# bentherien/point-cloud-reid

Measured on NVIDIA B200. Metric: pair scores/sec (PT-256 encode + all-pairs xcorr_eff match), higher is better.
Workload: dtype f16

## Files before the change

include/pcreid.h:

```cpp
#ifndef PCREID_H_
#define PCREID_H_

#ifdef __cplusplus
extern "C" {
#endif

#define PCREID_OK 0
#define PCREID_ERR_ARG 1
#define PCREID_ERR_LAUNCH 2
#define PCREID_ERR_UNSUPPORTED 3

int pcreid_abi_version(void);


int pcreid_fps(int b, int n, int m, const float* xyz, float* temp, int* idx, void* stream);
int pcreid_fps_with_dist(int b, int n, int m, const float* dist, float* temp, int* idx, void* stream);
int pcreid_fps_block_size(int n);
int pcreid_fps_torch(int b, int n, int m, const float* xyz, const int* start, int* idx, void* stream);
int pcreid_pairwise_sqdist(int b, int n, int m, int c, const float* a, const float* bm, float* out, int norm, void* stream);

int pcreid_knn(int b, int n, int m, int nsample, const float* xyz, const float* new_xyz, int* idx, float* dist2, void* stream);
int pcreid_knn_t(int b, int n, int m, int nsample, const float* xyz, const float* new_xyz, int* idx, float* dist2, void* stream);

int pcreid_ball_query(int b, int n, int m, float min_radius, float max_radius, int nsample,
// ... 70 lines not shown
                   int rows2, const float* X2, long long x2_bs, int ldx2,
                   int mode, float* out, long long ob, long long oc, void* stream);
int pcreid_cn_chanmax(int B, int C, int rows, const float* X, long long x_bs, int ldx, float* out, long long ob, long long on, void* stream);

int pcreid_sa_edge_mlp(int B, int C, int N, int S, int k, const float* P1, const float* Cc, const int* idx,
                       const float* W2, const float* b2, const float* W3, const float* b3, float* out, void* stream);

int pcreid_edge_build(int B, int C, int N, int S, int k, const float* P1, const float* Cc, const int* idx, float* out, void* stream);
int pcreid_seg_max(long long rows, int k, const float* x, float* out, void* stream);
int pcreid_seg_mean(long long rows, int k, const float* x, float* out, void* stream);

int pcreid_edge_gather_max(int B, int C, int N, int k, const float* P, const float* Q, const int* idx, int act,
                           float* out, long long o_bs, int ldo, void* stream);

int pcreid_pair_concat_head_tc(int T, int D, int E, int G, const float* A, const float* Bv, const float* Et, const float* Ed,
                               const void* W2img, const float* g1, const float* be1, const float* g2, const float* be2,
                               const float* w, float b0, const unsigned char* mask, float* out, int n_ctas, void* stream);
int pcreid_pair_concat_head(int T, int D, int E, int G, const float* A, const float* Bv, const float* Et, const float* Ed,
                            const float* W2, const float* g1, const float* be1, const float* g2, const float* be2,
                            const float* w, float b0, const unsigned char* mask, float* out, void* stream);

#define PCREID_FMT_BF16 0
#define PCREID_FMT_F16 1
int pcreid_pack_image(int B, int C, int N, const float* src, long long s_bs, int lds, int act, int fmt, void* dst, void* stream);
int pcreid_pack_image_bias(int B, int C, int N, const float* src, long long s_bs, int lds, const float* bias, int fmt, void* dst,
                           void* stream);
int pcreid_pack_b7(int B, const float* M, const float* ksum, int fmt, void* dst, void* stream);
int pcreid_pool_finish2(int P, int npts, const float* part, const float* bias , float* out, void* stream);
int pcreid_pair_p1a2(int n_units, int npts, int role, int fmt, float att_eps, const int* u_search, const int* u_templ,
                     const int* u_slot, const void* QF1, const void* H, const void* MK1, const void* W, void* A_out,
                     int n_ctas, void* stream);
int pcreid_pair_p1b_n(int n_units, int npts, int role, int fmt, float kv_scale, const int* u_search, const int* u_templ,
                      const int* u_slot, const void* PV, const void* W, void* A_out, void* B7_out, int n_ctas, void* stream);
int pcreid_pair_p2y(int n_units, int npts, int role, int fmt, float att_eps, const int* u_slot, const void* A_in, const void* B7_in,
                    const void* W, float* pool_part, int n_ctas, void* stream);

int pcreid_sa_edge_mlp_tc(int B, int C, int N, int S, int k, const float* P1, const float* Cc, const int* idx,
                          const float* W2img, const float* b2, const float* W3img, const float* b3, float* out,
                          int n_ctas, void* stream);

int pcreid_sa_edge_mlp_tc2(int B, int C, int N, int S, int k, const float* P1, const float* Cc, const int* idx,
                           const float* W2img, const float* b2, const float* W3img, const float* b3, float* out,
                           int out_pm, int n_sms, void* stream);

int pcreid_attn_front_blob_bytes(int C2, int DP, int NFP, int NF);
int pcreid_attn_front(int B, int S, int C2, int DP, int NFP, int NF, const float* xyz, const float* feat, long long f_bs, int ldf,
                      const float* wp0, const float* bp0, const float* bp2, const void* blob, float* out, long long o_bs, int ldo,
                      void* stream);
int pcreid_linattn_kv_img(int B, int S, int d, int H, const float* K, long long k_bs, int ldk, const float* V, long long v_bs, int ldv,
                          float* kvimg, float* ksum, void* stream);
int pcreid_attn_back_objects_per_tile(int rows, int D);
int pcreid_attn_back_blob_bytes(int D, int C1P, int CO, int qpre);
int pcreid_attn_back(int B, int rows, int D, int H, int C1, int CO, int res, int f1_pm, const float* feat1, long long f1_bs,
                     int ldf1, const float* q, long long q_bs, int ldq, const float* ksum, const float* kvimg, const float* g1,
                     const float* b1, const float* g2, const float* b2, const void* blob, float* out, long long o_bs, int ldo,
                     void* stream);

#ifdef __cplusplus
}
#endif
#endif
```

point-cloud-reid_b200/_lib.py:

```python
import ctypes
import os

_HERE = os.path.dirname(os.path.abspath(__file__))
LIB_PATH = os.path.join(_HERE, "libpcreid_sm100.so")
_lib = None

c_int, c_ll, c_float, c_vp = ctypes.c_int, ctypes.c_longlong, ctypes.c_float, ctypes.c_void_p


class LinearArgs(ctypes.Structure):
    _fields_ = [
        ("B", c_int), ("rows", c_int), ("CO", c_int), ("K1", c_int), ("K2", c_int),
        ("X1", c_vp), ("x1_bs", c_ll), ("ldx1", c_int), ("x1_pm", c_int), ("x1_map", c_vp),
        ("X2", c_vp), ("x2_bs", c_ll), ("ldx2", c_int), ("x2_pm", c_int), ("x2_map", c_vp),
        ("W1", c_vp), ("w1_bs", c_ll), ("w1_map", c_vp),
        ("W2", c_vp), ("w2_bs", c_ll),
        ("bias", c_vp),
        ("R", c_vp), ("r_bs", c_ll), ("ldr", c_int), ("r_map", c_vp), ("res_after_act", c_int),
        ("act", c_int),
        ("Y", c_vp), ("y_bs", c_ll), ("ldy", c_int), ("y_pm", c_int),
    ]


class NormArgs(ctypes.Structure):
# ... 29 lines not shown
    "pcreid_crop_gather": [c_int, c_int, c_int, c_vp, c_int, c_vp, c_vp, c_vp, c_vp, c_vp, c_vp],
    "pcreid_three_nn": [c_int, c_int, c_int, c_vp, c_vp, c_vp, c_vp, c_vp],
    "pcreid_three_interpolate": [c_int, c_int, c_int, c_int, c_vp, c_vp, c_vp, c_vp, c_vp],
    "pcreid_cn_linear": [ctypes.POINTER(LinearArgs), c_vp],
    "pcreid_cn_linear_tc": [ctypes.POINTER(LinearArgs), c_vp],
    "pcreid_cn_linear_tc2": [ctypes.POINTER(LinearArgs), c_vp, c_vp, c_int, c_vp],
    "pcreid_cn_linear_tma": [ctypes.POINTER(LinearArgs), c_ll, c_ll, c_ll, c_int, c_int, c_vp],
    "pcreid_cn_linear_tma_x3": [ctypes.POINTER(LinearArgs), c_vp, c_vp, c_ll, c_ll, c_ll, c_int, c_vp],
    "pcreid_cn_groupnorm": [ctypes.POINTER(NormArgs), c_vp],
    "pcreid_gn_res_relu_dot": [c_int, c_int, c_int, c_vp, c_int, c_vp, c_vp, c_vp, c_int, c_vp, c_float, c_vp, c_vp],
    "pcreid_attn_front_blob_bytes": [c_int, c_int, c_int, c_int],
    "pcreid_attn_front": [c_int, c_int, c_int, c_int, c_int, c_int, c_vp, c_vp, c_ll, c_int, c_vp, c_vp, c_vp, c_vp, c_vp, c_ll, c_int,
                          c_vp],
    "pcreid_linattn_kv_img": [c_int, c_int, c_int, c_int, c_vp, c_ll, c_int, c_vp, c_ll, c_int, c_vp, c_vp, c_vp],
    "pcreid_attn_back_objects_per_tile": [c_int, c_int],
    "pcreid_attn_back_blob_bytes": [c_int, c_int, c_int, c_int],
    "pcreid_attn_back": [c_int] * 8 + [c_vp, c_ll, c_int, c_vp, c_ll, c_int] + [c_vp] * 7 + [c_vp, c_ll, c_int, c_vp],
    "pcreid_linattn_kv": [c_int, c_int, c_int, c_int, c_vp, c_ll, c_int, c_vp, c_ll, c_int, c_vp, c_vp, c_vp],
    "pcreid_linattn_scale": [c_int, c_int, c_int, c_int, c_int, c_vp, c_ll, c_int, c_vp, c_vp, c_vp, c_vp, c_ll, c_int, c_vp],
    "pcreid_local_linattn": [c_int, c_int, c_int, c_int, c_int, c_vp, c_vp, c_vp, c_vp],
    "pcreid_cn_pool": [c_int, c_int, c_int, c_vp, c_ll, c_int, c_int, c_vp, c_ll, c_int, c_int, c_vp, c_ll, c_ll, c_vp],
    "pcreid_cn_chanmax": [c_int, c_int, c_int, c_vp, c_ll, c_int, c_vp, c_ll, c_ll, c_vp],
    "pcreid_sa_edge_mlp": [c_int, c_int, c_int, c_int, c_int, c_vp, c_vp, c_vp, c_vp, c_vp, c_vp, c_vp, c_vp, c_vp],
    "pcreid_edge_build": [c_int, c_int, c_int, c_int, c_int, c_vp, c_vp, c_vp, c_vp, c_vp],
    "pcreid_seg_max": [c_ll, c_int, c_vp, c_vp, c_vp],
    "pcreid_seg_mean": [c_ll, c_int, c_vp, c_vp, c_vp],
    "pcreid_edge_gather_max": [c_int, c_int, c_int, c_int, c_vp, c_vp, c_vp, c_int, c_vp, c_ll, c_int, c_vp],
    "pcreid_pack_image": [c_int, c_int, c_int, c_vp, c_ll, c_int, c_int, c_int, c_vp, c_vp],
    "pcreid_pack_image_bias": [c_int, c_int, c_int, c_vp, c_ll, c_int, c_vp, c_int, c_vp, c_vp],
    "pcreid_pack_b7": [c_int, c_vp, c_vp, c_int, c_vp, c_vp],
    "pcreid_pool_finish2": [c_int, c_int, c_vp, c_vp, c_vp, c_vp],
    "pcreid_pair_p1a2": [c_int, c_int, c_int, c_int, c_float] + [c_vp] * 8 + [c_int, c_vp],
    "pcreid_pair_p1b_n": [c_int, c_int, c_int, c_int, c_float] + [c_vp] * 7 + [c_int, c_vp],
    "pcreid_pair_p2y": [c_int, c_int, c_int, c_int, c_float] + [c_vp] * 5 + [c_int, c_vp],
    "pcreid_sa_edge_mlp_tc": [c_int, c_int, c_int, c_int, c_int] + [c_vp] * 8 + [c_int, c_vp],
    "pcreid_sa_edge_mlp_tc2": [c_int, c_int, c_int, c_int, c_int] + [c_vp] * 8 + [c_int, c_int, c_vp],
    "pcreid_pair_concat_head_tc": [c_int, c_int, c_int, c_int] + [c_vp] * 10 + [c_float, c_vp, c_vp, c_int, c_vp],
    "pcreid_pair_concat_head": [c_int, c_int, c_int, c_int] + [c_vp] * 10 + [c_float, c_vp, c_vp, c_vp],
}

ERRORS = {1: "PCREID_ERR_ARG (bad pointer/size)", 2: "PCREID_ERR_LAUNCH (CUDA launch failed)",
          3: "PCREID_ERR_UNSUPPORTED (shape outside the built kernels)"}


def exported_symbols():
    return sorted(_SIGS.keys())


def lib():
    global _lib
    if _lib is not None:
        return _lib
    if not os.path.exists(LIB_PATH):
        from . import build as _build
        _build.build_library()
    if not os.path.exists(LIB_PATH):
        raise RuntimeError(f"{LIB_PATH} is missing and could not be built: the CUDA extension is required "
                           "(no CPU fallback exists)")
    L = ctypes.CDLL(LIB_PATH)
    for name, argt in _SIGS.items():
        fn = getattr(L, name)
        fn.argtypes = argt
        fn.restype = c_int
    _lib = L
    return L

# ... 10 lines not shown
```

point-cloud-reid_b200/csrc/pair_common.cuh:

```cuda
#pragma once
#include "../../include/pcreid.h"
#include "common.cuh"
#include "tc_common.cuh"

namespace {


constexpr int IMG = 16384;
constexpr int NB7H = 80;
constexpr int B7_HEAD = (NB7H / 8) * 32 * 16;
constexpr int B7_BYTES = 2 * B7_HEAD;
constexpr int ONES_BYTES = 2 * 2048;
constexpr float LN_EPS = 1e-5f;

struct P1Args {
  int n_units, NT, role;
  int npts;
  float att_eps;
  float kv_scale;
  const int *u_search, *u_templ, *u_slot;
  const uint8_t *QF1, *H, *PV;
  const uint8_t* MK1;
  const uint8_t* W;
  uint8_t* A_out;
  uint8_t* B7_out;
};
struct P2Args {
  int n_units, NT, role;
  int npts;
  float att_eps;
  const int* u_slot;
  const uint8_t* A_in;
  const uint8_t* B7_in;
  const uint8_t* W;
  float* pool_part;
};

__device__ __forceinline__ float elu1(float x) { return x > 0.f ? x + 1.f : __expf(x); }

__device__ __forceinline__ uint4 ldg_early(const void* p) {
  uint4 v;
  asm volatile("ld.global.nc.L1::no_allocate.v4.u32 {%0,%1,%2,%3}, [%4];" : "=r"(v.x), "=r"(v.y), "=r"(v.z), "=r"(v.w) : "l"(p));
  return v;
}

__device__ __forceinline__ void prefetch_l2_16k(const uint8_t* img, int t) {
  asm volatile("prefetch.global.L2 [%0];" ::"l"(img + (size_t)t * 128));
}

__device__ __forceinline__ void copy_to_smem(uint8_t* dst, const uint8_t* __restrict__ src, int bytes, int t, int nthr) {
  for (int i = t * 16; i < bytes; i += nthr * 16) cp_async16(dst + i, src + i);
}

struct Opnd {
  uint64_t desc;
  uint32_t kstep;
};
__device__ __forceinline__ Opnd opnd(uint32_t addr, uint32_t lbo, uint32_t sbo, uint32_t kstep_bytes) {
// ... 42 lines not shown
  uint32_t tmem, tlane;
  uint64_t* bar;
  uint32_t par;
  __device__ __forceinline__ void sync() { tc::bar_sync(1 + gid, GX); }
  __device__ __forceinline__ void publish() { tc::fence_async_smem(); tc::tc_fence_before(); sync(); tc::tc_fence_after(); }
  __device__ __forceinline__ void wait() { tc::mbar_wait(bar, par); par ^= 1u; tc::tc_fence_after(); }
};

__device__ __forceinline__ void ld32_stats(uint32_t taddr, float (&o)[32], float& s, float& ss) {
#pragma unroll
  for (int half = 0; half < 2; ++half) {
    uint32_t r[16];
    tc::tmem_ld16(taddr + 16 * half, r);
    tc::tmem_ld_wait();
#pragma unroll
    for (int j = 0; j < 16; ++j) {
      const float v = __uint_as_float(r[j]);
      o[16 * half + j] = v;
      s += v;
      ss = fmaf(v, v, ss);
    }
  }
}

template <class F>
__device__ __forceinline__ void write_b7_row(const float (&M)[64], float ksum, int d, uint8_t* dst) {
  float lo[32], hi[32];
#pragma unroll
  for (int j = 0; j < 32; ++j) { lo[j] = M[j]; hi[j] = M[32 + j]; }
  write_b7_part<F>(lo, 0, ksum, true, d, dst);
  write_b7_part<F>(hi, 4, ksum, false, d, dst);
}

__device__ __forceinline__ void groupx_setup(GroupX& g, uint64_t* bars, uint32_t tmem_base) {
  const int warp_u = (int)tc::uniform(threadIdx.x >> 5);
  g.gid = warp_u / 4;
  g.t = threadIdx.x % GX;
  g.issuer = (warp_u % 4) == 0;
  g.tmem = tc::uniform(tmem_base) + g.gid * 160;
  g.tlane = g.tmem + ((uint32_t)((warp_u % 4) * 32) << 16);
  g.bar = bars + g.gid;
  g.par = 0;
}

}
```

point-cloud-reid_b200/csrc/pair_tc.cu:

```cuda
#include "pair_common.cuh"
#include <stdlib.h>

namespace {

constexpr int P1B_WKV = 0, P1B_WM = 16384, P1B_WBYTES = 24576;
constexpr int P1B_AIMG = 0, P1B_KFV = IMG, P1B_GBYTES = IMG + 2 * IMG + ONES_BYTES;

template <class F, int CS>
__global__ void __launch_bounds__(NGX * GX * CS, 1) pair_p1b_kernel(const P1Args a) {
  constexpr int GT = GX * CS, NTHR = NGX * GT;
  constexpr int QB = 4 / CS, CB = 8 / CS;
  extern __shared__ __align__(1024) uint8_t smem[];
  __shared__ uint64_t bars[2 * NGX];
  __shared__ uint32_t tmem_base_s;
  uint8_t* Wsm = smem;
  if (threadIdx.x == 0) {
    for (int i = 0; i < 2 * NGX; ++i) tc::mbar_init(&bars[i], 1);
    tc::fence_mbar_init();
  }
  if (threadIdx.x < 32) { tc::tmem_alloc(&tmem_base_s, 512); tc::tmem_relinquish(); }
  copy_to_smem(Wsm, a.W, P1B_WBYTES, threadIdx.x, NTHR);
  cp_async_commit();
  cp_async_wait<0>();
  tc::fence_async_smem();
  tc::tc_fence_before();
  __syncthreads();
  tc::tc_fence_after();
  const int warp_u = (int)tc::uniform(threadIdx.x >> 5);
  const int gid = warp_u / (4 * CS), wg = warp_u % (4 * CS), gt = threadIdx.x % GT;
  const int half = wg / 4;
  const int row = (wg % 4) * 32 + (threadIdx.x & 31);
  const bool issuer = wg == 0;
  const uint32_t tmem = tc::uniform(tmem_base_s) + gid * 160;
  const uint32_t tlane = tmem + ((uint32_t)((wg % 4) * 32) << 16);
  uint64_t* bar = bars + gid;
  uint32_t par = 0;
  auto gsync = [&]() { tc::bar_sync(1 + gid, GT); };
  auto publish = [&]() { tc::fence_async_smem(); tc::tc_fence_before(); gsync(); tc::tc_fence_after(); };
// ... 450 lines not shown
```

point-cloud-reid_b200/csrc/pair_tc2.cu:

```cuda
#include "pair_common.cuh"
#include <stdlib.h>

namespace {

constexpr int Q1A_W0 = 0, Q1A_W2 = 18 * 2048, Q1A_LN = Q1A_W2 + 16384, Q1A_WBYTES = Q1A_LN + 256;
constexpr int Q1A_ONES = Q1A_WBYTES;
constexpr int Q1A_QXA = 0, Q1A_H = IMG, Q1A_MK1 = 2 * IMG, Q1A_GBYTES = 2 * IMG + B7_BYTES;
constexpr int Q2_WQ = 0, Q2_W0 = 8192, Q2_W2 = Q2_W0 + 18 * 2048, Q2_LN = Q2_W2 + 16384, Q2_WBYTES = Q2_LN + 256;
constexpr int Q2_ONES = Q2_WBYTES;
constexpr int Q2_R1 = 0, Q2_B7 = 2 * IMG, Q2_GBYTES = Q2_B7 + B7_BYTES;

__device__ __forceinline__ float u2f(uint32_t u) { return __uint_as_float(u); }

template <class F>
__device__ __forceinline__ void tmem_ones(const GroupX& g) {
  if (g.gid == 0) {
    uint32_t w[32];
#pragma unroll
    for (int j = 0; j < 32; ++j) w[j] = 0u;
    w[0] = F::ONE_LO;
    tc::tmem_st32(g.tlane + 480, w);
    tc::tmem_st_wait();
  }
  tc::tc_fence_before();
// ... 194 lines not shown
          for (int ks = 0; ks < 8; ++ks)
            tc::umma_f16_ts(g.tmem + 64, g.tmem + 8 * ks, oW2.desc + (uint64_t)(ks * oW2.kstep), id64, ks > 0 ? 1u : 0u);
          tc::umma_commit(g.bar);
        }
        __syncwarp();
      }
      {
        uint4 sdH[8];
        load_side<8>(sdH, a.H + ti * IMG, 0, row);
        g.wait();
        uint32_t x0[32], x1[32];
        const float rstd = rsqrtf(ld64_sumsq(g.tlane + 64, x0, x1) * (1.f / 64.f) + LN_EPS);
        if (tile + 1 < a.NT) start_tile(ti + 1, te);
        else if (u + 1 < u1) start_tile((size_t)so_next * a.NT, te_next);
        uint8_t* orow = a.A_out + (((size_t)slot * 2 + a.role) * a.NT + tile) * IMG + row * 16;
#pragma unroll
        for (int hh = 0; hh < 2; ++hh) {
          uint32_t (&x)[32] = hh == 0 ? x0 : x1;
#pragma unroll
          for (int c = 0; c < 4; ++c) {
            const uint4 rs = sdH[4 * hh + c];
            const float4 ga = g2v[8 * hh + 2 * c], gb = g2v[8 * hh + 2 * c + 1];
            uint32_t w[4];
            w[0] = F::pack(fmaf(u2f(x[c * 8 + 0]) * rstd, ga.x, F::lo(rs.x)), fmaf(u2f(x[c * 8 + 1]) * rstd, ga.y, F::hi(rs.x)));
            w[1] = F::pack(fmaf(u2f(x[c * 8 + 2]) * rstd, ga.z, F::lo(rs.y)), fmaf(u2f(x[c * 8 + 3]) * rstd, ga.w, F::hi(rs.y)));
            w[2] = F::pack(fmaf(u2f(x[c * 8 + 4]) * rstd, gb.x, F::lo(rs.z)), fmaf(u2f(x[c * 8 + 5]) * rstd, gb.y, F::hi(rs.z)));
            w[3] = F::pack(fmaf(u2f(x[c * 8 + 6]) * rstd, gb.z, F::lo(rs.w)), fmaf(u2f(x[c * 8 + 7]) * rstd, gb.w, F::hi(rs.w)));
            *reinterpret_cast<uint4*>(orow + (4 * hh + c) * 2048) = make_uint4(w[0], w[1], w[2], w[3]);
          }
        }
      }
      tc::tc_fence_before();
    }
  }
  cp_async_wait<0>();
  tc::tc_fence_before();
  __syncthreads();
  if (threadIdx.x < 32) tc::tmem_dealloc(tmem_base_s, 512);
}

template <class F, bool XT>
__global__ void __launch_bounds__(NGX * GX, 1) pair_p2y_kernel(const P2Args a) {
  extern __shared__ __align__(1024) uint8_t smem[];
  __shared__ uint64_t bars[NGX];
  __shared__ uint32_t tmem_base_s;
  __shared__ __align__(16) float comb[NGX][4][2][64];
  uint8_t* Wsm = smem;
  const float4* g2v = reinterpret_cast<const float4*>(Wsm + Q2_LN);
  if (threadIdx.x == 0) {
    for (int i = 0; i < NGX; ++i) tc::mbar_init(&bars[i], 1);
    tc::fence_mbar_init();
  }
  if (threadIdx.x < 32) { tc::tmem_alloc(&tmem_base_s, 512); tc::tmem_relinquish(); }
  copy_to_smem(Wsm, a.W, Q2_WBYTES, threadIdx.x, NGX * GX);
  cp_async_commit();
  if (threadIdx.x < 256)
    reinterpret_cast<uint4*>(smem + Q2_ONES)[threadIdx.x] = threadIdx.x < 128 ? make_uint4(F::ONE_LO, 0, 0, 0) : make_uint4(0, 0, 0, 0);
  cp_async_wait<0>();
  tc::fence_async_smem();
  tc::tc_fence_before();
  __syncthreads();
  tc::tc_fence_after();
  GroupX g;
  groupx_setup(g, bars, tmem_base_s);
  const uint32_t t_ones = tc::uniform(tmem_base_s) + 480;
  if constexpr (XT) { tmem_ones<F>(g); __syncthreads(); tc::tc_fence_after(); }
// ... 231 lines not shown
  const int chunk = (int)((idx / 128) % nch);
  const int tile = (int)((idx / (128LL * nch)) % nt);
  const long long b = idx / (128LL * nch * nt);
  if (b >= B) return;
  const float* s = src + b * s_bs + (size_t)(chunk * 8) * lds + tile * 128 + row;
  uint32_t w[4] = {0u, 0u, 0u, 0u};
  if (tile * 128 + row < N) {
#pragma unroll
    for (int j = 0; j < 4; ++j)
      w[j] = F::pack(s[(size_t)(2 * j) * lds] + bias[chunk * 8 + 2 * j], s[(size_t)(2 * j + 1) * lds] + bias[chunk * 8 + 2 * j + 1]);
  }
  *reinterpret_cast<uint4*>(dst + (((size_t)b * nt + tile) * nch + chunk) * 2048 + row * 16) = make_uint4(w[0], w[1], w[2], w[3]);
}

}

static int x_tmem_mask() {
  static const int m = [] { const char* e = getenv("PCREID_X_TMEM"); return e ? atoi(e) : 3; }();
  return m;
}

template <class F, bool XT>
static int launch_p1a2_x(const P1Args& a, int grid, cudaStream_t st) {
  const int smem = Q1A_ONES + 4096 + NGX * Q1A_GBYTES;
  cudaFuncSetAttribute(pair_p1a2_kernel<F, XT>, cudaFuncAttributeMaxDynamicSharedMemorySize, smem);
  pair_p1a2_kernel<F, XT><<<grid, NGX * GX, smem, st>>>(a);
  return pcreid_launch_status();
}
template <class F>
static int launch_p1a2(const P1Args& a, int grid, cudaStream_t st) {
  return (x_tmem_mask() & 1) ? launch_p1a2_x<F, true>(a, grid, st) : launch_p1a2_x<F, false>(a, grid, st);
}

template <class F, bool XT>
static int launch_p2y_x(const P2Args& a, int grid, cudaStream_t st) {
  const int smem = Q2_ONES + 4096 + NGX * Q2_GBYTES;
  cudaFuncSetAttribute(pair_p2y_kernel<F, XT>, cudaFuncAttributeMaxDynamicSharedMemorySize, smem);
  pair_p2y_kernel<F, XT><<<grid, NGX * GX, smem, st>>>(a);
  return pcreid_launch_status();
}
template <class F>
static int launch_p2y(const P2Args& a, int grid, cudaStream_t st) {
  return (x_tmem_mask() & 2) ? launch_p2y_x<F, true>(a, grid, st) : launch_p2y_x<F, false>(a, grid, st);
}

extern "C" {

int pcreid_pack_image_bias(int B, int C, int N, const float* src, long long s_bs, int lds, const float* bias, int fmt, void* dst,
                           void* stream) {
  if (B <= 0) return PCREID_OK;
  if (!src || !dst || !bias || C % 8 || N <= 0 || (fmt != PCREID_FMT_BF16 && fmt != PCREID_FMT_F16)) return PCREID_ERR_ARG;
  const long long per = 128LL * (C / 8) * ((N + 127) / 128);
  const unsigned grid = (unsigned)((per * B + 255) / 256);
  if (fmt == PCREID_FMT_F16)
    pack_image_bias_kernel<tc::OpF16><<<grid, 256, 0, (cudaStream_t)stream>>>(B, C, N, src, s_bs, lds, bias, (uint8_t*)dst);
  else
    pack_image_bias_kernel<tc::OpBF16><<<grid, 256, 0, (cudaStream_t)stream>>>(B, C, N, src, s_bs, lds, bias, (uint8_t*)dst);
  return pcreid_launch_status();
}

int pcreid_pool_finish2(int P, int npts, const float* part, const float* bias, float* out, void* stream) {
  if (P <= 0) return PCREID_OK;
  if (!part || !out) return PCREID_ERR_ARG;
  pool_finish2_kernel<<<(unsigned)((P + 31) / 32), 256, 0, (cudaStream_t)stream>>>(P, npts, part, bias, out);
  return pcreid_launch_status();
}

int pcreid_pair_p1a2(int n_units, int npts, int role, int fmt, float att_eps, const int* u_search, const int* u_templ, const int* u_slot,
                     const void* QF1, const void* H, const void* MK1, const void* W, void* A_out, int n_ctas, void* stream) {
  if (n_units <= 0) return PCREID_OK;
  if (!u_search || !u_templ || !u_slot || !QF1 || !H || !MK1 || !W || !A_out || npts <= 0 ||
      (fmt != PCREID_FMT_BF16 && fmt != PCREID_FMT_F16))
    return PCREID_ERR_ARG;
  const int NT = (npts + 127) / 128;
  P1Args a{n_units, NT, role, npts, att_eps, 1.f, u_search, u_templ, u_slot, (const uint8_t*)QF1, (const uint8_t*)H,
           nullptr, (const uint8_t*)MK1, (const uint8_t*)W, (uint8_t*)A_out, nullptr};
  int grid = n_ctas > 0 ? n_ctas : 148;
  if (grid * NGX > n_units) grid = (n_units + NGX - 1) / NGX;
  return fmt == PCREID_FMT_F16 ? launch_p1a2<tc::OpF16>(a, grid, (cudaStream_t)stream) : launch_p1a2<tc::OpBF16>(a, grid, (cudaStream_t)stream);
}

int pcreid_pair_p2y(int n_units, int npts, int role, int fmt, float att_eps, const int* u_slot, const void* A_in, const void* B7_in,
                    const void* W, float* pool_part, int n_ctas, void* stream) {
  if (n_units <= 0) return PCREID_OK;
  if (!u_slot || !A_in || !B7_in || !W || !pool_part || npts <= 0 || (fmt != PCREID_FMT_BF16 && fmt != PCREID_FMT_F16)) return PCREID_ERR_ARG;
  const int NT = (npts + 127) / 128;
  P2Args a{n_units, NT, role, npts, att_eps, u_slot, (const uint8_t*)A_in, (const uint8_t*)B7_in, (const uint8_t*)W, pool_part};
  int grid = n_ctas > 0 ? n_ctas : 148;
  if (grid * NGX > n_units) grid = (n_units + NGX - 1) / NGX;
  return fmt == PCREID_FMT_F16 ? launch_p2y<tc::OpF16>(a, grid, (cudaStream_t)stream) : launch_p2y<tc::OpBF16>(a, grid, (cudaStream_t)stream);
}

}
```

point-cloud-reid_b200/csrc/rowops.cu:

```cuda
#include "../../include/pcreid.h"
#include "common.cuh"

namespace {

constexpr int TR = 128;
constexpr int KC = 16;
constexpr int NTHR = 256;

template <int TN>
struct TileCols { static constexpr int value = 16 * TN; };

template <int TN>
__device__ __forceinline__ void fma_chunk(const float* __restrict__ Xs, const float* __restrict__ Ws, int tx, int ty,
                                          float (&acc)[8][TN]) {
  constexpr int TC = TileCols<TN>::value;
#pragma unroll
  for (int kk = 0; kk < KC; ++kk) {
    const float4 a0 = *reinterpret_cast<const float4*>(Xs + kk * TR + tx * 4);
    const float4 a1 = *reinterpret_cast<const float4*>(Xs + kk * TR + 64 + tx * 4);
    const float a[8] = {a0.x, a0.y, a0.z, a0.w, a1.x, a1.y, a1.z, a1.w};
    float w[TN];
    {
      const float4 w0 = *reinterpret_cast<const float4*>(Ws + kk * TC + ty * 4);
      w[0] = w0.x; w[1] = w0.y; w[2] = w0.z; w[3] = w0.w;
// ... 664 lines not shown
  for (int g0 = 0; g0 < CPW; g0 += CG) {
    float s = 0.f;
#pragma unroll
    for (int i = 0; i < CG; ++i) s += y[g0 + i];
    const float mean = s / (float)CG;
    float v = 0.f;
#pragma unroll
    for (int i = 0; i < CG; ++i) { float dd = y[g0 + i] - mean; v = fmaf(dd, dd, v); }
    const float rstd = rsqrtf(v / (float)CG + 1e-5f);
#pragma unroll
    for (int i = 0; i < CG; ++i) {
      const int c = wq * CPW + g0 + i;
      float r = 0.f;
      if (valid) r = c < E ? __ldg(Et + (size_t)t * E + c) : __ldg(Ed + (size_t)d * E + (c - E));
      const float o = fmaxf((y[g0 + i] - mean) * rstd * __ldg(g2 + c) + __ldg(be2 + c) + r, 0.f);
      part = fmaf(o, __ldg(w + c), part);
    }
  }
  red[wq][lane] = part;
  __syncthreads();
  if (wq == 0 && valid) {
    float s = b0;
#pragma unroll
    for (int i = 0; i < 8; ++i) s += red[i][lane];
    if (mask && !mask[(size_t)t * D + d]) s = 0.f;
    out[(size_t)t * D + d] = s;
  }
}

}

extern "C" {

int pcreid_abi_version(void) { return 1; }

int pcreid_cn_linear(const pcreid_linear_args* p, void* stream) {
  if (!p) return PCREID_ERR_ARG;
  pcreid_linear_args a = *p;
  if (a.B <= 0 || a.rows <= 0 || a.CO <= 0) return PCREID_OK;
  if (a.K1 <= 0 || !a.X1 || !a.W1 || !a.Y) return PCREID_ERR_ARG;
  if (a.K2 > 0 && (!a.X2 || !a.W2)) return PCREID_ERR_ARG;
  if (a.B > 65535 * 32) return PCREID_ERR_UNSUPPORTED;
  cudaStream_t st = (cudaStream_t)stream;
  const int zmax = 65535;
  for (int b0 = 0; b0 < a.B; b0 += zmax) {
    pcreid_linear_args s = a;
    s.B = (a.B - b0 < zmax) ? a.B - b0 : zmax;
    if (b0) {
      if (s.x1_map) s.x1_map += b0; else s.X1 += (size_t)b0 * s.x1_bs;
      if (s.K2 > 0) { if (s.x2_map) s.x2_map += b0; else s.X2 += (size_t)b0 * s.x2_bs; s.W2 += (size_t)b0 * s.w2_bs; }
      if (s.w1_map) s.w1_map += b0; else s.W1 += (size_t)b0 * s.w1_bs;
      if (s.R) { if (s.r_map) s.r_map += b0; else s.R += (size_t)b0 * s.r_bs; }
      s.Y += (size_t)b0 * s.y_bs;
    }
    auto a16 = [](const void* q) { return (reinterpret_cast<uintptr_t>(q) & 15) == 0; };
    const bool pack = s.rows < TR && TR % s.rows == 0 && s.rows % 4 == 0 && s.B > 1 && !s.x1_map && !s.x2_map && !s.w1_map && !s.r_map &&
                      !s.x1_pm && !s.x2_pm && !s.y_pm && s.w1_bs == 0 && (s.K2 == 0 || s.w2_bs == 0) && s.CO % 4 == 0 &&
                      a16(s.X1) && s.ldx1 % 4 == 0 && s.x1_bs % 4 == 0 && a16(s.W1) && a16(s.Y) && s.ldy % 4 == 0 && s.y_bs % 4 == 0 &&
                      (s.K2 == 0 || (a16(s.X2) && s.ldx2 % 4 == 0 && s.x2_bs % 4 == 0 && a16(s.W2))) &&
                      (!s.R || (a16(s.R) && s.ldr % 4 == 0 && s.r_bs % 4 == 0));
    if (pack) {
      const int nz = ceil_div(s.B, TR / s.rows);
      if (a.CO > 64) cn_linear_kernel<8, true><<<dim3(1, ceil_div(a.CO, 128), nz), NTHR, 0, st>>>(s);
      else cn_linear_kernel<4, true><<<dim3(1, 1, nz), NTHR, 0, st>>>(s);
    } else if (a.CO > 64) {
      dim3 grid(ceil_div(a.rows, TR), ceil_div(a.CO, 128), s.B);
      cn_linear_kernel<8><<<grid, NTHR, 0, st>>>(s);
// ... 209 lines not shown
```

point-cloud-reid_b200/models/fused_pairs.py:

```python
import math
import os

import torch

from .. import kernels as K
from .. import torch_ops as _T
from ._packing import kmajor

IMG = 16384
B7_BYTES = int(os.environ.get("PCREID_B7_BYTES", 10240))
FMT_BF16, FMT_F16 = 0, 1
LN2H = 0.693359375
LN2B = 0.69140625
ATT_EPS = 1e-6


def _center_out(w):
    w = w.detach().float()
    return w - w.mean(0, keepdim=True)


_OPS = _T.ops


def _w_image(w, dtype):
    N, Kd = w.shape
    return w.detach().to(dtype).view(N, Kd // 8, 8).permute(1, 0, 2).contiguous().view(torch.uint8).flatten()


def _f32_bytes(*ts):
    return torch.cat([t.detach().float().flatten() for t in ts]).contiguous().view(torch.uint8)


def supported(model, n_points):
    X1, X2 = model.cross_stage1, model.cross_stage2
    return (model.match_type == 'xcorr_eff' and model.combine == 'point-cat' and model.pool_type == 'both'
            and X1 is not None and X2 is not None and X1.q_proj.weight.shape == (64, 64) and X1.nhead == 2
            and X2.q_proj.weight.shape == (64, 64) and X2.nhead == 2 and n_points >= 1)


class ObjectPack:
    __slots__ = ("n", "npts", "fmt", "QF1", "H", "PV", "MK1")


class FusedXcorr:
    def __init__(self, model, fmt=FMT_BF16):
        self.model = model
# ... 81 lines not shown
            ksum = ksum * sc
        o.MK1 = torch.empty((B, B7_BYTES), device=h.device, dtype=torch.uint8)
        _OPS.pack_b7(B, M, ksum, self.fmt, o.MK1)
        return o

    def _dense_units(self, dev, r0, nrows, Dn, by_search, b_by_search):
        key = (str(dev), r0, nrows, Dn, by_search, b_by_search)
        capturing = torch.cuda.is_current_stream_capturing()
        hit = None if capturing else self._units.get(key)
        if hit is not None:
            return hit
        P = nrows * Dn
        u = torch.arange(P, device=dev, dtype=torch.int32)
        t_of, d_of = r0 + u % nrows, u // nrows
        c = lambda *xs: tuple(x.contiguous() for x in xs)
        lists_s = (c(r0 + u // Dn, u % Dn, u),
                   c(u // nrows, r0 + u % nrows, (u % nrows) * Dn + u // nrows))
        lists_t = (c(t_of, d_of, (t_of - r0) * Dn + d_of),
                   c(u % Dn, r0 + u // Dn, u))
        out = (lists_s if by_search else lists_t, lists_s if b_by_search else lists_t)
        if not capturing:
            if len(self._units) >= 64:
                self._units.pop(next(iter(self._units)))
            self._units[key] = out
        return out

    def match(self, pt, pd, ti, dj, debug=None, dense=None):
        assert pt.npts == pd.npts, "fused matcher expects equal point counts on both sides"
        assert pt.fmt == self.fmt and pd.fmt == self.fmt, "object packs were prepared for another operand format"
        self._weights()
        dev = pt.H.device
        if self.n_ctas is None or self._n_ctas_dev != dev:
            self.n_ctas, self._n_ctas_dev = torch.cuda.get_device_properties(dev).multi_processor_count, dev
        by_search = False
        b_by_search = os.environ.get("PCREID_P1B_ORDER", "search") == "search"
        if dense is not None:
            r0, nrows, Dn = dense
            P = nrows * Dn
            unit_lists, unit_lists_b = self._dense_units(dev, r0, nrows, Dn, by_search, b_by_search)
        else:
            P = ti.numel()
            ti, dj = ti.long(), dj.long()
            unit_lists = None
        NT, N = (pt.npts + 127) // 128, pt.npts
        A = torch.empty((P, 2, NT, IMG), device=dev, dtype=torch.uint8)
        B7 = torch.empty((P, 2, B7_BYTES), device=dev, dtype=torch.uint8)
        part = torch.empty((P, 2, 128), device=dev, dtype=torch.float32)
        sc = self.kv_scale(N)
        for role, (srch, tmpl, ps, pm) in enumerate(((ti, dj, pt, pd), (dj, ti, pd, pt))):
            if unit_lists is not None:
                us, ut, sl = unit_lists[role]
                bs, bt, bl = unit_lists_b[role]
            else:
                order = torch.argsort(tmpl, stable=True)
                us, ut, sl = srch[order].int().contiguous(), tmpl[order].int().contiguous(), order.int().contiguous()
                bs, bt, bl = us, ut, sl
                if b_by_search:
                    order = torch.argsort(srch, stable=True)
                    bs, bt, bl = srch[order].int().contiguous(), tmpl[order].int().contiguous(), order.int().contiguous()
            e0 = self._tick()
            _OPS.pair_p1a2(P, N, role, self.fmt, ATT_EPS * sc, us, ut, sl, ps.QF1, ps.H, pm.MK1, self._w1a2, A, self.n_ctas)
            self._tock("pair_p1a2_kernel", e0, P)
            e0 = self._tick()
            _OPS.pair_p1b_n(P, N, role, self.fmt, sc, bs, bt, bl, ps.PV, self._w1b2, A, B7, self.n_ctas)
            self._tock("pair_p1b_kernel" if os.environ.get("PCREID_P1B") == "1" else "pair_p1b2_kernel", e0, P)
        slots = torch.arange(P, device=dev, dtype=torch.int32)
        pooled = torch.empty((1, 128, P), device=dev, dtype=torch.float32)
        for role in (0, 1):
            e0 = self._tick()
            _OPS.pair_p2y(P, N, role, self.fmt, ATT_EPS * sc, slots, A, B7, self._w2y, part, self.n_ctas)
            self._tock("pair_p2y_kernel", e0, P)
        _OPS.pool_finish2(P, N, part, self._b2_2, pooled)
        if debug is not None:
            debug.update(A=A, B7=B7, part=part, pooled=pooled)
        return self.model._head_cn(pooled)


def decode_image(img, dtype=torch.bfloat16):
    x = img.contiguous().view(dtype).float().transpose(-1, -2)
    return x.reshape(*x.shape[:-3], x.shape[-3] * 8, 128)


def decode_b7(img, dtype=torch.bfloat16):
    x = img.contiguous().view(dtype).float().reshape(*img.shape[:-1], 2, 10, 32, 8)
    nd = x.dim()
    return x.permute(*range(nd - 3), nd - 2, nd - 3, nd - 1).reshape(*img.shape[:-1], 2, 32, 80)
```

Before: 7.333 million.

## Fuse pair phase-1 attention and KV kernels into one persistent kernel

Adds a fused pair_p1 kernel that runs the p1a2 cross-attention/LN stage and the p1b K/V linear-attention stage back to back per unit in one launch. The A rows it has just written are reread from global memory (mostly L2) rather than passing through a second kernel, and both weight images stay resident in shared memory. It becomes the default path unless split-mode env vars are set, and units are now ordered by template for both stages. This removes one launch per role and the second kernel's weight load and scheduling, at the cost of larger shared memory and TMEM use per CTA and a longer serial per-unit pipeline.

```diff
diff --git a/include/pcreid.h b/include/pcreid.h
--- a/include/pcreid.h
+++ b/include/pcreid.h
@@ -126,6 +126,10 @@
                      int n_ctas, void* stream);
 int pcreid_pair_p1b_n(int n_units, int npts, int role, int fmt, float kv_scale, const int* u_search, const int* u_templ,
                       const int* u_slot, const void* PV, const void* W, void* A_out, void* B7_out, int n_ctas, void* stream);
+int pcreid_pair_p1(int n_units, int npts, int role, int fmt, float att_eps, float kv_scale, const int* u_search, const int* u_templ,
+                   const int* u_slot, const void* QF1, const void* H, const void* PV, const void* MK1, const void* Wa, const void* Wb,
+                   void* A_out, void* B7_out, int n_ctas, void* stream);
+int pcreid_pair_p1_budget(int* tmem_cols);
 int pcreid_pair_p2y(int n_units, int npts, int role, int fmt, float att_eps, const int* u_slot, const void* A_in, const void* B7_in,
                     const void* W, float* pool_part, int n_ctas, void* stream);
 
diff --git a/point-cloud-reid_b200/_lib.py b/point-cloud-reid_b200/_lib.py
--- a/point-cloud-reid_b200/_lib.py
+++ b/point-cloud-reid_b200/_lib.py
@@ -85,6 +85,8 @@
     "pcreid_pool_finish2": [c_int, c_int, c_vp, c_vp, c_vp, c_vp],
     "pcreid_pair_p1a2": [c_int, c_int, c_int, c_int, c_float] + [c_vp] * 8 + [c_int, c_vp],
     "pcreid_pair_p1b_n": [c_int, c_int, c_int, c_int, c_float] + [c_vp] * 7 + [c_int, c_vp],
+    "pcreid_pair_p1": [c_int, c_int, c_int, c_int, c_float, c_float] + [c_vp] * 11 + [c_int, c_vp],
+    "pcreid_pair_p1_budget": [c_vp],
     "pcreid_pair_p2y": [c_int, c_int, c_int, c_int, c_float] + [c_vp] * 5 + [c_int, c_vp],
     "pcreid_sa_edge_mlp_tc": [c_int, c_int, c_int, c_int, c_int] + [c_vp] * 8 + [c_int, c_vp],
     "pcreid_sa_edge_mlp_tc2": [c_int, c_int, c_int, c_int, c_int] + [c_vp] * 8 + [c_int, c_int, c_vp],
diff --git a/point-cloud-reid_b200/csrc/pair_common.cuh b/point-cloud-reid_b200/csrc/pair_common.cuh
--- a/point-cloud-reid_b200/csrc/pair_common.cuh
+++ b/point-cloud-reid_b200/csrc/pair_common.cuh
@@ -12,6 +12,7 @@
 constexpr int B7_BYTES = 2 * B7_HEAD;
 constexpr int ONES_BYTES = 2 * 2048;
 constexpr float LN_EPS = 1e-5f;
+constexpr int P1B_WKV = 0, P1B_WM = 16384, P1B_WBYTES = 24576;
 
 struct P1Args {
   int n_units, NT, role;
@@ -24,6 +25,7 @@
   const uint8_t* W;
   uint8_t* A_out;
   uint8_t* B7_out;
+  const uint8_t* Wb;
 };
 struct P2Args {
   int n_units, NT, role;
@@ -132,12 +134,12 @@
   write_b7_part<F>(hi, 4, ksum, false, d, dst);
 }
 
-__device__ __forceinline__ void groupx_setup(GroupX& g, uint64_t* bars, uint32_t tmem_base) {
+__device__ __forceinline__ void groupx_setup(GroupX& g, uint64_t* bars, uint32_t tmem_base, int tmem_cols = 160) {
   const int warp_u = (int)tc::uniform(threadIdx.x >> 5);
   g.gid = warp_u / 4;
   g.t = threadIdx.x % GX;
   g.issuer = (warp_u % 4) == 0;
-  g.tmem = tc::uniform(tmem_base) + g.gid * 160;
+  g.tmem = tc::uniform(tmem_base) + g.gid * tmem_cols;
   g.tlane = g.tmem + ((uint32_t)((warp_u % 4) * 32) << 16);
   g.bar = bars + g.gid;
   g.par = 0;
diff --git a/point-cloud-reid_b200/csrc/pair_tc.cu b/point-cloud-reid_b200/csrc/pair_tc.cu
--- a/point-cloud-reid_b200/csrc/pair_tc.cu
+++ b/point-cloud-reid_b200/csrc/pair_tc.cu
@@ -3,7 +3,6 @@
 
 namespace {
 
-constexpr int P1B_WKV = 0, P1B_WM = 16384, P1B_WBYTES = 24576;
 constexpr int P1B_AIMG = 0, P1B_KFV = IMG, P1B_GBYTES = IMG + 2 * IMG + ONES_BYTES;
 
 template <class F, int CS>
diff --git a/point-cloud-reid_b200/csrc/pair_tc2.cu b/point-cloud-reid_b200/csrc/pair_tc2.cu
--- a/point-cloud-reid_b200/csrc/pair_tc2.cu
+++ b/point-cloud-reid_b200/csrc/pair_tc2.cu
@@ -250,6 +250,295 @@
       }
       tc::tc_fence_before();
     }
+  }
+  cp_async_wait<0>();
+  tc::tc_fence_before();
+  __syncthreads();
+  if (threadIdx.x < 32) tc::tmem_dealloc(tmem_base_s, 512);
+}
+
+constexpr int P1_TG = 168, P1_KVC = 64, P1_AC = 136;
+constexpr int P1_WB = Q1A_WBYTES, P1_G0 = P1_WB + P1B_WBYTES;
+constexpr int P1_QXA = 0, P1_H = IMG, P1_ONES = 2 * IMG, P1_MK1 = P1_ONES + 4096, P1_GBYTES = P1_MK1 + B7_BYTES;
+constexpr int P1_SMEM = P1_G0 + NGX * P1_GBYTES;
+static_assert(NGX * P1_TG <= 512, "tensor-memory columns");
+static_assert(P1_SMEM + 1024 <= 227 * 1024, "dynamic + static shared memory");
+
+template <class F>
+__global__ void __launch_bounds__(NGX * GX, 1) pair_p1_kernel(const P1Args a) {
+  extern __shared__ __align__(1024) uint8_t smem[];
+  __shared__ uint64_t bars[NGX];
+  __shared__ uint32_t tmem_base_s;
+  __shared__ float ksum_s[NGX][64];
+  uint8_t* Wsm = smem;
+  const float4* g2v = reinterpret_cast<const float4*>(Wsm + Q1A_LN);
+  if (threadIdx.x == 0) {
+    for (int i = 0; i < NGX; ++i) tc::mbar_init(&bars[i], 1);
+    tc::fence_mbar_init();
+  }
+  if (threadIdx.x < 32) { tc::tmem_alloc(&tmem_base_s, 512); tc::tmem_relinquish(); }
+  copy_to_smem(Wsm, a.W, Q1A_WBYTES, threadIdx.x, NGX * GX);
+  copy_to_smem(Wsm + P1_WB, a.Wb, P1B_WBYTES, threadIdx.x, NGX * GX);
+  cp_async_commit();
+  {
+    uint4* ones = reinterpret_cast<uint4*>(smem + P1_G0 + (threadIdx.x / GX) * P1_GBYTES + P1_ONES);
+    ones[threadIdx.x % GX] = make_uint4(F::ONE_LO, 0, 0, 0);
+    ones[GX + threadIdx.x % GX] = make_uint4(0, 0, 0, 0);
+  }
+  cp_async_wait<0>();
+  tc::fence_async_smem();
+  tc::tc_fence_before();
+  __syncthreads();
+  tc::tc_fence_after();
+  GroupX g;
+  groupx_setup(g, bars, tmem_base_s, P1_TG);
+  const int wq = (int)tc::uniform(threadIdx.x >> 5) % 4, lane = threadIdx.x & 31;
+  uint8_t* G = smem + P1_G0 + g.gid * P1_GBYTES;
+  uint8_t* QXa = G + P1_QXA;
+  uint8_t* Hs = G + P1_H;
+  uint8_t* MK1 = G + P1_MK1;
+  uint8_t* KfV = G;
+  const uint32_t sG = tc::smem_u32(G), sW = tc::smem_u32(Wsm);
+  const uint32_t id80 = tc::instr_desc(128, NB7H, F::FMT, tc::MAJOR_K, tc::MAJOR_MN);
+  const uint32_t id128 = tc::instr_desc(128, 128, F::FMT, tc::MAJOR_K, tc::MAJOR_K);
+  const uint32_t id64 = tc::instr_desc(128, 64, F::FMT, tc::MAJOR_K, tc::MAJOR_K);
+  const uint32_t idkv = tc::instr_desc(64, 72, F::FMT, tc::MAJOR_MN, tc::MAJOR_MN);
+  const Opnd oQXa = A_IMG(sG + P1_QXA), oOnes = A_IMG(sG + P1_ONES), oMK1 = B7_IMG(sG + P1_MK1), oW0 = W_IMG(sW + Q1A_W0, 128),
+             oW2 = W_IMG(sW + Q1A_W2, 64), oWk = W_IMG(sW + P1_WB + P1B_WKV, 128), oWv = W_IMG(sW + P1_WB + P1B_WKV + 64 * 16, 128),
+             oWm = W_IMG(sW + P1_WB + P1B_WM, 64), oKf = opnd(sG, 128u, 2048u, 256u), oVones = opnd(sG + 8 * 2048, 128u, 2048u, 256u),
+             oBd = A_IMG(sG);
+  const int row = g.t;
+  const int ngroups = gridDim.x * NGX, gg = blockIdx.x * NGX + g.gid;
+  const int u0 = (int)((long long)a.n_units * gg / ngroups), u1 = (int)((long long)a.n_units * (gg + 1) / ngroups);
+  int cur_templ = -1;
+  int so_next = u0 < u1 ? a.u_search[u0] : 0, te_next = u0 < u1 ? a.u_templ[u0] : 0, slot_next = u0 < u1 ? a.u_slot[u0] : 0;
+  auto fill = [&](size_t ti_, int te_) {
+    copy_to_smem(QXa, a.QF1 + ti_ * IMG, IMG, g.t, GX);
+    copy_to_smem(Hs, a.H + ti_ * IMG, IMG, g.t, GX);
+    if (te_ != cur_templ) { copy_to_smem(MK1, a.MK1 + (size_t)te_ * B7_BYTES, B7_BYTES, g.t, GX); cur_templ = te_; }
+    cp_async_commit();
+  };
+  auto start_g1 = [&]() {
+    cp_async_wait<0>();
+    g.publish();
+    if (g.issuer) { if (tc::elect_one()) { issue_attn(g.tmem, oQXa, oMK1, id80); tc::umma_commit(g.bar); } __syncwarp(); }
+  };
+  if (u0 < u1) fill((size_t)so_next * a.NT, te_next);
+  for (int u = u0; u < u1; ++u) {
+    const int so = so_next, te = te_next, slot = slot_next;
+    if (u + 1 < u1) { so_next = a.u_search[u + 1]; te_next = a.u_templ[u + 1]; slot_next = a.u_slot[u + 1]; }
+    uint8_t* const a_unit = a.A_out + ((size_t)slot * 2 + a.role) * a.NT * IMG;
+    start_g1();
+    if (u + 1 < u1) {
+      prefetch_l2_16k(a.QF1 + (size_t)so_next * a.NT * IMG, g.t);
+      prefetch_l2_16k(a.H + (size_t)so_next * a.NT * IMG, g.t);
+      if (te_next != te && g.t < B7_BYTES / 128) prefetch_l2_16k(a.MK1 + (size_t)te_next * B7_BYTES, g.t);
+    }
+    for (int tile = 0; tile < a.NT; ++tile) {
+      const size_t ti = (size_t)so * a.NT + tile;
+      g.wait();
+      epi_attn_norm<F, true>(g.tlane, nullptr, a.att_eps);
+      g.publish();
+      if (g.issuer) {
+        if (tc::elect_one()) {
+#pragma unroll
+          for (int ks = 0; ks < 4; ++ks)
+            tc::umma_f16_ts(g.tmem, g.tmem + 128 + 8 * ks, oW0.desc + (uint64_t)(ks * oW0.kstep), id128, ks > 0 ? 1u : 0u);
+#pragma unroll
+          for (int ks = 4; ks < 8; ++ks)
+            tc::umma_f16(g.tmem, oQXa.desc + (uint64_t)(ks * oQXa.kstep), oW0.desc + (uint64_t)(ks * oW0.kstep), id128, 1u);
+          tc::umma_f16(g.tmem, oOnes.desc, oW0.desc + (uint64_t)(8 * oW0.kstep), id128, 1u);
+          tc::umma_commit(g.bar);
+        }
+        __syncwarp();
+      }
+      g.wait();
+      if (tile + 1 < a.NT) {
+        copy_to_smem(QXa, a.QF1 + (ti + 1) * IMG, IMG, g.t, GX);
+        copy_to_smem(Hs, a.H + (ti + 1) * IMG, IMG, g.t, GX);
+        cp_async_commit();
+      }
+#pragma unroll
+      for (int b = 0; b < 2; ++b) {
+        uint32_t r0[32], r1[32], w[32];
+        tc::tmem_ld32(g.tlane + 64 * b, r0);
+        tc::tmem_ld32(g.tlane + 64 * b + 32, r1);
+        tc::tmem_ld_wait();
+#pragma unroll
+        for (int j = 0; j < 16; ++j) {
+          w[j] = F::pack_relu(u2f(r0[2 * j]), u2f(r0[2 * j + 1]));
+          w[16 + j] = F::pack_relu(u2f(r1[2 * j]), u2f(r1[2 * j + 1]));
+        }
+        tc::tmem_st32(g.tlane + 32 * b, w);
+      }
+      tc::tmem_st_wait();
+      tc::tc_fence_before();
+      g.sync();
+      tc::tc_fence_after();
+      if (g.issuer) {
+        if (tc::elect_one()) {
+#pragma unroll
+          for (int ks = 0; ks < 8; ++ks)
+            tc::umma_f16_ts(g.tmem + 64, g.tmem + 8 * ks, oW2.desc + (uint64_t)(ks * oW2.kstep), id64, ks > 0 ? 1u : 0u);
+          tc::umma_commit(g.bar);
+        }
+        __syncwarp();
+      }
+      {
+        uint4 sdH[8];
+        load_side<8>(sdH, a.H + ti * IMG, 0, row);
+        g.wait();
+        uint32_t x0[32], x1[32];
+        const float rstd = rsqrtf(ld64_sumsq(g.tlane + 64, x0, x1) * (1.f / 64.f) + LN_EPS);
+        if (tile + 1 < a.NT) start_g1();
+        uint8_t* orow = a_unit + (size_t)tile * IMG + row * 16;
+#pragma unroll
+        for (int hh = 0; hh < 2; ++hh) {
+          uint32_t (&x)[32] = hh == 0 ? x0 : x1;
+#pragma unroll
+          for (int c = 0; c < 4; ++c) {
+            const uint4 rs = sdH[4 * hh + c];
+            const float4 ga = g2v[8 * hh + 2 * c], gb = g2v[8 * hh + 2 * c + 1];
+            uint32_t w[4];
+            w[0] = F::pack(fmaf(u2f(x[c * 8 + 0]) * rstd, ga.x, F::lo(rs.x)), fmaf(u2f(x[c * 8 + 1]) * rstd, ga.y, F::hi(rs.x)));
+            w[1] = F::pack(fmaf(u2f(x[c * 8 + 2]) * rstd, ga.z, F::lo(rs.y)), fmaf(u2f(x[c * 8 + 3]) * rstd, ga.w, F::hi(rs.y)));
+            w[2] = F::pack(fmaf(u2f(x[c * 8 + 4]) * rstd, gb.x, F::lo(rs.z)), fmaf(u2f(x[c * 8 + 5]) * rstd, gb.y, F::hi(rs.z)));
+            w[3] = F::pack(fmaf(u2f(x[c * 8 + 6]) * rstd, gb.z, F::lo(rs.w)), fmaf(u2f(x[c * 8 + 7]) * rstd, gb.w, F::hi(rs.w)));
+            *reinterpret_cast<uint4*>(orow + (4 * hh + c) * 2048) = make_uint4(w[0], w[1], w[2], w[3]);
+          }
+        }
+      }
+      tc::tc_fence_before();
+    }
+    uint32_t areg[32];
+    auto load_row = [&](int tile) {
+#pragma unroll
+      for (int c = 0; c < 8; ++c) {
+        asm volatile("ld.global.v4.u32 {%0,%1,%2,%3}, [%4];"
+                     : "=r"(areg[4 * c]), "=r"(areg[4 * c + 1]), "=r"(areg[4 * c + 2]), "=r"(areg[4 * c + 3])
+                     : "l"(a_unit + (size_t)tile * IMG + c * 2048 + row * 16) : "memory");
+      }
+    };
+    load_row(0);
+    for (int tile = 0; tile < a.NT; ++tile) {
+      const size_t ti = (size_t)so * a.NT + tile;
+      tc::tmem_st32(g.tlane + P1_AC, areg);
+      tc::tmem_st_wait();
+      tc::tc_fence_before();
+      g.sync();
+      tc::tc_fence_after();
+      if (g.issuer) {
+        if (tc::elect_one()) {
+#pragma unroll
+          for (int ks = 0; ks < 4; ++ks) tc::umma_f16_ts(g.tmem, g.tmem + P1_AC + 8 * ks, oWk.desc + (uint64_t)(ks * oWk.kstep), id64, ks > 0 ? 1u : 0u);
+          tc::umma_commit(g.bar);
+        }
+        __syncwarp();
+      }
+      if (tile + 1 < a.NT) load_row(tile + 1);
+      g.wait();
+      {
+        const bool keep = tile * 128 + row < a.npts;
+#pragma unroll
+        for (int q = 0; q < 4; ++q) {
+          uint32_t r[16];
+          tc::tmem_ld16(g.tlane + 16 * q, r);
+          tc::tmem_ld_wait();
+#pragma unroll
+          for (int c = 0; c < 2; ++c) {
+            uint32_t w[4];
+#pragma unroll
+            for (int j = 0; j < 4; ++j)
+              w[j] = keep ? F::elu1(__uint_as_float(r[c * 8 + 2 * j]), __uint_as_float(r[c * 8 + 2 * j + 1])) : 0u;
+            *reinterpret_cast<uint4*>(KfV + (2 * q + c) * 2048 + row * 16) = make_uint4(w[0], w[1], w[2], w[3]);
+          }
+        }
+      }
+      tc::tc_fence_before();
+      g.sync();
+      tc::tc_fence_after();
+      if (g.issuer) {
+        if (tc::elect_one()) {
+#pragma unroll
+          for (int ks = 0; ks < 4; ++ks) tc::umma_f16_ts(g.tmem, g.tmem + P1_AC + 8 * ks, oWv.desc + (uint64_t)(ks * oWv.kstep), id64, ks > 0 ? 1u : 0u);
+          tc::umma_commit(g.bar);
+        }
+        __syncwarp();
+      }
+      {
+        uint4 sdPV[8];
+        load_side<8>(sdPV, a.PV + ti * IMG, 0, row);
+        g.wait();
+#pragma unroll
+        for (int q = 0; q < 4; ++q) {
+          uint32_t r[16];
+          tc::tmem_ld16(g.tlane + 16 * q, r);
+          tc::tmem_ld_wait();
+#pragma unroll
+          for (int c = 0; c < 2; ++c) {
+            const uint4 s4 = sdPV[2 * q + c];
+            const uint32_t sw[4] = {s4.x, s4.y, s4.z, s4.w};
+            uint32_t w[4];
+#pragma unroll
+            for (int j = 0; j < 4; ++j)
+              w[j] = F::add(__uint_as_float(r[c * 8 + 2 * j]), __uint_as_float(r[c * 8 + 2 * j + 1]), sw[j]);
+            *reinterpret_cast<uint4*>(KfV + (8 + 2 * q + c) * 2048 + row * 16) = make_uint4(w[0], w[1], w[2], w[3]);
+          }
+        }
+      }
+      g.publish();
+      if (g.issuer) {
+        if (tc::elect_one()) { issue_gemm<8>(g.tmem + P1_KVC, oKf, oVones, idkv, tile > 0); tc::umma_commit(g.bar); }
+        __syncwarp();
+      }
+      g.wait();
+    }
+    {
+      float kv[64];
+      uint32_t r8[8];
+#pragma unroll
+      for (int q = 0; q < 4; ++q) {
+        uint32_t r[16];
+        tc::tmem_ld16(g.tlane + P1_KVC + 16 * q, r);
+        tc::tmem_ld_wait();
+#pragma unroll
+        for (int j = 0; j < 16; ++j) kv[16 * q + j] = __uint_as_float(r[j]) * a.kv_scale;
+      }
+      tc::tmem_ld8(g.tlane + P1_KVC + 64, r8);
+      tc::tmem_ld_wait();
+      if (lane < 16) {
+        const int i = 16 * wq + lane, hd = i >> 5;
+        ksum_s[g.gid][i] = __uint_as_float(r8[0]) * a.kv_scale;
+#pragma unroll
+        for (int c = 0; c < 8; ++c) {
+          uint32_t w[4];
+#pragma unroll
+          for (int j = 0; j < 4; ++j) w[j] = ((c >> 2) == hd) ? F::pack(kv[c * 8 + 2 * j], kv[c * 8 + 2 * j + 1]) : 0u;
+          *reinterpret_cast<uint4*>(G + c * 2048 + i * 16) = make_uint4(w[0], w[1], w[2], w[3]);
+        }
+      }
+    }
+    if (row >= 64) {
+#pragma unroll
+      for (int c = 0; c < 8; ++c) *reinterpret_cast<uint4*>(G + c * 2048 + row * 16) = make_uint4(0, 0, 0, 0);
+    }
+    g.publish();
+    if (g.issuer) { if (tc::elect_one()) { issue_gemm<4>(g.tmem, oBd, oWm, id64, false); tc::umma_commit(g.bar); } __syncwarp(); }
+    g.wait();
+    if (u + 1 < u1) fill((size_t)so_next * a.NT, te_next);
+    if (row < 64) {
+      float kv[64];
+#pragma unroll
+      for (int q = 0; q < 4; ++q) {
+        uint32_t r[16];
+        tc::tmem_ld16(g.tlane + 16 * q, r);
+        tc::tmem_ld_wait();
+#pragma unroll
+        for (int j = 0; j < 16; ++j) kv[16 * q + j] = __uint_as_float(r[j]);
+      }
+      write_b7_row<F>(kv, ksum_s[g.gid][row], row, a.B7_out + ((size_t)slot * 2 + a.role) * B7_BYTES);
+    }
+    tc::tc_fence_before();
   }
   cp_async_wait<0>();
   tc::tc_fence_before();
@@ -547,6 +836,13 @@
   return (x_tmem_mask() & 1) ? launch_p1a2_x<F, true>(a, grid, st) : launch_p1a2_x<F, false>(a, grid, st);
 }
 
+template <class F>
+static int launch_p1(const P1Args& a, int grid, cudaStream_t st) {
+  cudaFuncSetAttribute(pair_p1_kernel<F>, cudaFuncAttributeMaxDynamicSharedMemorySize, P1_SMEM);
+  pair_p1_kernel<F><<<grid, NGX * GX, P1_SMEM, st>>>(a);
+  return pcreid_launch_status();
+}
+
 template <class F, bool XT>
 static int launch_p2y_x(const P2Args& a, int grid, cudaStream_t st) {
   const int smem = Q2_ONES + 4096 + NGX * Q2_GBYTES;
@@ -595,6 +891,26 @@
   return fmt == PCREID_FMT_F16 ? launch_p1a2<tc::OpF16>(a, grid, (cudaStream_t)stream) : launch_p1a2<tc::OpBF16>(a, grid, (cudaStream_t)stream);
 }
 
+int pcreid_pair_p1(int n_units, int npts, int role, int fmt, float att_eps, float kv_scale, const int* u_search, const int* u_templ,
+                   const int* u_slot, const void* QF1, const void* H, const void* PV, const void* MK1, const void* Wa, const void* Wb,
+                   void* A_out, void* B7_out, int n_ctas, void* stream) {
+  if (n_units <= 0) return PCREID_OK;
+  if (!u_search || !u_templ || !u_slot || !QF1 || !H || !PV || !MK1 || !Wa || !Wb || !A_out || !B7_out || npts <= 0 ||
+      (fmt != PCREID_FMT_BF16 && fmt != PCREID_FMT_F16))
+    return PCREID_ERR_ARG;
+  const int NT = (npts + 127) / 128;
+  P1Args a{n_units, NT, role, npts, att_eps, kv_scale, u_search, u_templ, u_slot, (const uint8_t*)QF1, (const uint8_t*)H,
+           (const uint8_t*)PV, (const uint8_t*)MK1, (const uint8_t*)Wa, (uint8_t*)A_out, (uint8_t*)B7_out, (const uint8_t*)Wb};
+  int grid = n_ctas > 0 ? n_ctas : 148;
+  if (grid * NGX > n_units) grid = (n_units + NGX - 1) / NGX;
+  return fmt == PCREID_FMT_F16 ? launch_p1<tc::OpF16>(a, grid, (cudaStream_t)stream) : launch_p1<tc::OpBF16>(a, grid, (cudaStream_t)stream);
+}
+
+int pcreid_pair_p1_budget(int* tmem_cols) {
+  if (tmem_cols) *tmem_cols = NGX * P1_TG;
+  return P1_SMEM;
+}
+
 int pcreid_pair_p2y(int n_units, int npts, int role, int fmt, float att_eps, const int* u_slot, const void* A_in, const void* B7_in,
                     const void* W, float* pool_part, int n_ctas, void* stream) {
   if (n_units <= 0) return PCREID_OK;
diff --git a/point-cloud-reid_b200/csrc/rowops.cu b/point-cloud-reid_b200/csrc/rowops.cu
--- a/point-cloud-reid_b200/csrc/rowops.cu
+++ b/point-cloud-reid_b200/csrc/rowops.cu
@@ -720,7 +720,7 @@
 
 extern "C" {
 
-int pcreid_abi_version(void) { return 1; }
+int pcreid_abi_version(void) { return 2; }
 
 int pcreid_cn_linear(const pcreid_linear_args* p, void* stream) {
   if (!p) return PCREID_ERR_ARG;
diff --git a/point-cloud-reid_b200/models/fused_pairs.py b/point-cloud-reid_b200/models/fused_pairs.py
--- a/point-cloud-reid_b200/models/fused_pairs.py
+++ b/point-cloud-reid_b200/models/fused_pairs.py
@@ -13,6 +13,12 @@
 LN2H = 0.693359375
 LN2B = 0.69140625
 ATT_EPS = 1e-6
+
+
+def split_phase1():
+    e = os.environ
+    return (e.get("PCREID_PHASE1") == "split" or "PCREID_P1B" in e or "PCREID_P1B_ORDER" in e
+            or ("PCREID_X_TMEM" in e and not int(e["PCREID_X_TMEM"]) & 1))
 
 
 def _center_out(w):
@@ -160,8 +166,9 @@
         dev = pt.H.device
         if self.n_ctas is None or self._n_ctas_dev != dev:
             self.n_ctas, self._n_ctas_dev = torch.cuda.get_device_properties(dev).multi_processor_count, dev
+        split = split_phase1()
         by_search = False
-        b_by_search = os.environ.get("PCREID_P1B_ORDER", "search") == "search"
+        b_by_search = split and os.environ.get("PCREID_P1B_ORDER", "search") == "search"
         if dense is not None:
             r0, nrows, Dn = dense
             P = nrows * Dn
@@ -186,6 +193,12 @@
                 if b_by_search:
                     order = torch.argsort(srch, stable=True)
                     bs, bt, bl = srch[order].int().contiguous(), tmpl[order].int().contiguous(), order.int().contiguous()
+            if not split:
+                e0 = self._tick()
+                _OPS.pair_p1(P, N, role, self.fmt, ATT_EPS * sc, sc, us, ut, sl, ps.QF1, ps.H, ps.PV, pm.MK1, self._w1a2, self._w1b2, A, B7,
+                             self.n_ctas)
+                self._tock("pair_p1_kernel", e0, P)
+                continue
             e0 = self._tick()
             _OPS.pair_p1a2(P, N, role, self.fmt, ATT_EPS * sc, us, ut, sl, ps.QF1, ps.H, pm.MK1, self._w1a2, A, self.n_ctas)
             self._tock("pair_p1a2_kernel", e0, P)
```

After: 7.396 million, median of 6. About the same (+0.9%).
